# nikolovjovan/exblas

Measured on AMD Instinct MI355X. Metric: ExSUM fp64 Gelem/s at n=2^28 (bit-exact vs CPU superaccumulator/MPFR), higher is better.
Workload: dtype f64; 1 GPU; ExSUM n=2^28 fp64 ill_cond(c=1e+32), fpe=8 early_exit=True, 1xMI355X, inputs resident in HBM, steps rotate over 4 distinct vectors; n_total=268435456, fpe=8, early_exit=True, parallelism=single

## Files before the change

exblas_amd/csrc/blas1.hip:

```cpp
#include "superacc.hip.h"
#include "fpe.hip.h"
#include "exblas_internal.h"
#include <hip/hip_ext.h>

namespace exb {

constexpr int BLOCK = 256;
constexpr int WAVES = BLOCK / 64;
constexpr int U = 4;

template <int N, bool EE, int COPIES, int CNT, int ZM = 0>
__device__ __forceinline__ void fpe_absorb(double (&a)[N > 0 ? N : 1], double (&x)[CNT], int from,
                                           long long *col, unsigned &flags)
{
    LdsSink<COPIES> sink{col, flags};
    fpe_absorb_sink<N, EE, CNT, LdsSink<COPIES>, ZM>(a, x, from, sink);
}

template <int N, int COPIES>
__device__ __forceinline__ void fpe_flush(double (&a)[N > 0 ? N : 1], long long *col, unsigned &flags)
{
    LdsSink<COPIES> sink{col, flags};
    fpe_flush_sink<N>(a, sink);
}

template <int COPIES>
__device__ __forceinline__ void block_epilogue(long long *s_acc, unsigned flags, long long *gacc,
                                               unsigned *gflags, int ngroups)
{
    __shared__ unsigned s_flags;
    if (threadIdx.x == 0) s_flags = 0;
    __syncthreads();
    if (flags) atomicOr(&s_flags, flags);
    long long *g = gacc + (size_t)(blockIdx.x % ngroups) * NL;
    for (int l = threadIdx.x; l < NL; l += BLOCK) {
        long long sum = 0;
#pragma unroll
        for (int w = 0; w < WAVES; ++w)
#pragma unroll
            for (int c = 0; c < COPIES; ++c) sum += s_acc[(w * NL + l) * COPIES + c];
        if (sum != 0) atomicAdd((unsigned long long *)&g[l], (unsigned long long)sum);
    }
    __syncthreads();
    if (threadIdx.x == 0 && s_flags) atomicOr(gflags, s_flags);
}

template <int N, bool EE, int COPIES>
__global__ void __launch_bounds__(BLOCK) k_exsum(const double *__restrict__ a, long long n,
                                                 long long *__restrict__ gacc,
                                                 unsigned *__restrict__ gflags, int ngroups)
{
    __shared__ long long s_acc[WAVES * NL * COPIES];
    auto zero_lds = [&]() {
        for (int i = threadIdx.x; i < WAVES * NL * COPIES; i += BLOCK) s_acc[i] = 0;
        __syncthreads();
    };
    const int wave = threadIdx.x >> 6, lane = threadIdx.x & 63;
    long long *col = s_acc + wave * NL * COPIES + (lane & (COPIES - 1));
    unsigned flags = 0;
    double fpe[N > 0 ? N : 1];
#pragma unroll
    for (int i = 0; i < (N > 0 ? N : 1); ++i) fpe[i] = 0.0;

    const long long head = (((uintptr_t)a & 8u) && n > 0) ? 1 : 0;
    const d2_t *v = (const d2_t *)(a + head);
    const long long nv = (n - head) >> 1;
    constexpr long long TILE = (long long)BLOCK * U;
    const long long ntiles = nv / TILE;
    LdsSink<COPIES> sinkm{col, flags};
    Bypass bypass;

    long long t = blockIdx.x;
    if (t < ntiles) {
        d2_t r0[U], r1[U];
        auto fill = [&](long long tile, d2_t (&r)[U]) {
            const d2_t *p = v + (tile < ntiles ? tile : ntiles - 1) * TILE + threadIdx.x;
#pragma unroll
            for (int u = 0; u < U; ++u) r[u] = ld2(p + u * BLOCK);
        };
        auto absorb = [&](d2_t (&r)[U]) {
            double x[2 * U];
#pragma unroll
            for (int u = 0; u < U; ++u) {
                x[2 * u] = r[u].x;
                x[2 * u + 1] = r[u].y;
            }
            fpe_absorb_adaptive<N, EE, 2 * U, LdsSink<COPIES>>(fpe, x, sinkm, bypass);
        };
        fill(t, r0);
        zero_lds();
        for (;;) {
            fill(t + gridDim.x, r1);
            absorb(r0);
            t += gridDim.x;
            if (t >= ntiles) break;
            fill(t + gridDim.x, r0);
            absorb(r1);
            t += gridDim.x;
            if (t >= ntiles) break;
        }
    } else {
        zero_lds();
    }
    for (long long i = ntiles * TILE + (long long)blockIdx.x * BLOCK + threadIdx.x; i < nv;
         i += (long long)gridDim.x * BLOCK) {
        d2_t r = v[i];
        double x[2] = {r.x, r.y};
        fpe_absorb<N, false, COPIES, 2>(fpe, x, 0, col, flags);
    }
    if (blockIdx.x == 0 && threadIdx.x == 0) {
        if (head) lds_add<COPIES>(col, a[0], flags);
        if ((n - head) & 1) lds_add<COPIES>(col, a[n - 1], flags);
    }
    fpe_flush<N, COPIES>(fpe, col, flags);
    block_epilogue<COPIES>(s_acc, flags, gacc, gflags, ngroups);
}

template <int N, bool EE, int COPIES>
__global__ void __launch_bounds__(BLOCK) k_exsum_strided(const double *__restrict__ a, long long n,
                                                         long long inca, long long *__restrict__ gacc,
                                                         unsigned *__restrict__ gflags, int ngroups)
{
    __shared__ long long s_acc[WAVES * NL * COPIES];
    for (int i = threadIdx.x; i < WAVES * NL * COPIES; i += BLOCK) s_acc[i] = 0;
    __syncthreads();
    const int wave = threadIdx.x >> 6, lane = threadIdx.x & 63;
    long long *col = s_acc + wave * NL * COPIES + (lane & (COPIES - 1));
    unsigned flags = 0;
    double fpe[N > 0 ? N : 1];
#pragma unroll
    for (int i = 0; i < (N > 0 ? N : 1); ++i) fpe[i] = 0.0;
    const long long T = (long long)gridDim.x * BLOCK;
    for (long long i = (long long)blockIdx.x * BLOCK + threadIdx.x; i < n; i += 4 * T) {
        double x[4];
#pragma unroll
        for (int u = 0; u < 4; ++u) x[u] = i + u * T < n ? a[(i + u * T) * inca] : 0.0;
        fpe_absorb<N, false, COPIES, 4>(fpe, x, 0, col, flags);
    }
    fpe_flush<N, COPIES>(fpe, col, flags);
    block_epilogue<COPIES>(s_acc, flags, gacc, gflags, ngroups);
}

template <int N, bool EE, int COPIES, int ZM>
__global__ void __launch_bounds__(BLOCK) k_exdot(const double *__restrict__ a, const double *__restrict__ b,
                                                 long long n, long long *__restrict__ gacc,
                                                 unsigned *__restrict__ gflags, int ngroups)
{
    __shared__ long long s_acc[WAVES * NL * COPIES];
    auto zero_lds = [&]() {
        for (int i = threadIdx.x; i < WAVES * NL * COPIES; i += BLOCK) s_acc[i] = 0;
        __syncthreads();
    };
    const int wave = threadIdx.x >> 6, lane = threadIdx.x & 63;
    long long *col = s_acc + wave * NL * COPIES + (lane & (COPIES - 1));
    unsigned flags = 0;
    LdsSink<COPIES> sink{col, flags};
    long long *const lo_acc = low_acc_of(gflags), *const hi_acc = high_acc_of(gflags);
    double fpe[N > 0 ? N : 1];
#pragma unroll
    for (int i = 0; i < (N > 0 ? N : 1); ++i) fpe[i] = 0.0;

    const d2_t *va = (const d2_t *)a, *vb = (const d2_t *)b;
    const long long nv = n >> 1;
    Bypass bypass;
    constexpr long long TILE = (long long)BLOCK * U;
    const long long ntiles = nv / TILE;
    long long t = blockIdx.x;
    d2_t ra[U], rb[U];
    if (t < ntiles) {
        const long long base = t * TILE + threadIdx.x;
#pragma unroll
        for (int u = 0; u < U; ++u) {
            ra[u] = ld2(va + base + u * BLOCK);
            rb[u] = ld2(vb + base + u * BLOCK);
        }
    }
    zero_lds();
    if (t < ntiles) {
        d2_t rc[U], rd[U];
        auto fill = [&](long long tile, d2_t (&pa)[U], d2_t (&pb)[U]) {
            const long long base = (tile < ntiles ? tile : ntiles - 1) * TILE + threadIdx.x;
#pragma unroll
            for (int u = 0; u < U; ++u) {
                pa[u] = ld2(va + base + u * BLOCK);
                pb[u] = ld2(vb + base + u * BLOCK);
            }
        };
        auto absorb = [&](d2_t (&pa)[U], d2_t (&pb)[U]) {
            double x[2 * U], e[2 * U];
#pragma unroll
            for (int u = 0; u < U; ++u) {
                x[2 * u] = two_prod(pa[u].x, pb[u].x, e[2 * u]);
                x[2 * u + 1] = two_prod(pa[u].y, pb[u].y, e[2 * u + 1]);
            }
            if (!prod_range_divert<2 * U>(fpe[0], x, e, sink, lo_acc, hi_acc, [&](int j) { return j & 1 ? pa[j >> 1].y : pa[j >> 1].x; },
                                              [&](int j) { return j & 1 ? pb[j >> 1].y : pb[j >> 1].x; }))
                fpe_absorb_prod_adaptive<N, EE, 2 * U, LdsSink<COPIES>, ZM, false>(fpe, x, e, sink, bypass);
        };
        for (;;) {
            fill(t + gridDim.x, rc, rd);
            absorb(ra, rb);
            t += gridDim.x;
            if (t >= ntiles) break;
            fill(t + gridDim.x, ra, rb);
            absorb(rc, rd);
            t += gridDim.x;
            if (t >= ntiles) break;
        }
    }
    for (long long i = ntiles * TILE + (long long)blockIdx.x * BLOCK + threadIdx.x; i < nv;
         i += (long long)gridDim.x * BLOCK) {
        d2_t ra = va[i], rb = vb[i];
        double x[2], e[2];
        x[0] = two_prod(ra.x, rb.x, e[0]);
        x[1] = two_prod(ra.y, rb.y, e[1]);
        if (!prod_range_divert<2>(fpe[0], x, e, sink, lo_acc, hi_acc, [&](int j) { return j ? ra.y : ra.x; }, [&](int j) { return j ? rb.y : rb.x; }))
            fpe_absorb_prod<N, false, 2, LdsSink<COPIES>, 0, false>(fpe, x, e, sink);
    }
    if (blockIdx.x == 0 && threadIdx.x == 0 && (n & 1)) {
        double x1[1], e1[1];
        x1[0] = two_prod(a[n - 1], b[n - 1], e1[0]);
        if (!prod_range_divert<1>(fpe[0], x1, e1, sink, lo_acc, hi_acc, [&](int) { return a[n - 1]; }, [&](int) { return b[n - 1]; }))
            sink_product(sink, x1[0], e1[0]);
    }
    fpe_flush<N, COPIES>(fpe, col, flags);
    block_epilogue<COPIES>(s_acc, flags, gacc, gflags, ngroups);
}

template <int N, bool EE, int COPIES>
__global__ void __launch_bounds__(BLOCK) k_exdot_strided(const double *__restrict__ a, long long inca,
                                                         const double *__restrict__ b, long long incb,
                                                         long long n, long long *__restrict__ gacc,
                                                         unsigned *__restrict__ gflags, int ngroups)
{
    __shared__ long long s_acc[WAVES * NL * COPIES];
    for (int i = threadIdx.x; i < WAVES * NL * COPIES; i += BLOCK) s_acc[i] = 0;
    __syncthreads();
    const int wave = threadIdx.x >> 6, lane = threadIdx.x & 63;
    long long *col = s_acc + wave * NL * COPIES + (lane & (COPIES - 1));
    unsigned flags = 0;
    LdsSink<COPIES> sink{col, flags};
    long long *const lo_acc = low_acc_of(gflags), *const hi_acc = high_acc_of(gflags);
    double fpe[N > 0 ? N : 1];
#pragma unroll
    for (int i = 0; i < (N > 0 ? N : 1); ++i) fpe[i] = 0.0;
    const long long T = (long long)gridDim.x * BLOCK;
    for (long long i = (long long)blockIdx.x * BLOCK + threadIdx.x; i < n; i += 4 * T) {
        double va[4], vb[4], x[4], e[4];
#pragma unroll
        for (int u = 0; u < 4; ++u) {
            const bool in = i + u * T < n;
            va[u] = in ? a[(i + u * T) * inca] : 0.0;
            vb[u] = in ? b[(i + u * T) * incb] : 0.0;
        }
#pragma unroll
        for (int u = 0; u < 4; ++u) x[u] = two_prod(va[u], vb[u], e[u]);
        if (!prod_range_divert<4>(fpe[0], x, e, sink, lo_acc, hi_acc, [&](int j) { return va[j]; }, [&](int j) { return vb[j]; }))
            fpe_absorb_prod<N, false, 4, LdsSink<COPIES>, 0, false>(fpe, x, e, sink);
    }
    fpe_flush<N, COPIES>(fpe, col, flags);
    block_epilogue<COPIES>(s_acc, flags, gacc, gflags, ngroups);
}

__global__ void __launch_bounds__(64) k_finalize(long long *sets, int nsets, int set_stride, unsigned *gflags,
                                                 unsigned flags_or, int zero_sets, long long *out,
                                                 const long long *ext_in, long long *ext_out)
{
    const int lane = threadIdx.x;
    unsigned flags = flags_or;
    if (gflags) flags |= *gflags;
    if (set_stride >= SET_WORDS) {
        for (int g = 0; g < nsets; ++g)
        {
            for (int k = 0; k < 3; ++k)
                if (sets[(size_t)g * set_stride + NL + k] != 0) flags |= (1u << k);
            const long long pw = sets[(size_t)g * set_stride + NL + 3];
            if (pw & 0xffff) flags |= FLAG_PUNDER;
            if (pw >> 16) flags |= FLAG_POVER;
        }
    }
    long long lo0 = 0, hi0 = 0, lo1 = 0, hi1 = 0;
    for (int g0 = 0; g0 < nsets; g0 += 16) {
        long long t0[16], t1[16];
#pragma unroll
        for (int k = 0; k < 16; ++k) {
            const bool ok = g0 + k < nsets;
            const long long *p = sets + (size_t)(ok ? g0 + k : 0) * set_stride;
            t0[k] = ok ? __builtin_nontemporal_load(p + lane) : 0;
            t1[k] = (ok && lane < NL - 64) ? __builtin_nontemporal_load(p + 64 + lane) : 0;
        }
#pragma unroll
        for (int k = 0; k < 16; ++k) {
            lo0 += t0[k] & 0xffffffffll;
            hi0 += t0[k] >> 32;
            if (lane == NL - 65) {
                lo1 += t1[k];
            } else {
                lo1 += t1[k] & 0xffffffffll;
                hi1 += t1[k] >> 32;
            }
        }
    }
    long long in0 = __shfl_up(hi0, 1), in1 = __shfl_up(hi1, 1);
    const long long h63 = __shfl(hi0, 63);
    if (lane == 0) { in0 = 0; in1 = h63; }
    long long v0 = lo0 + in0, v1 = (lane < NL - 64) ? lo1 + in1 : 0;
    if (zero_sets) {
        for (int i = lane; i < nsets * set_stride; i += 64) sets[i] = 0;
        if (lane == 0 && gflags) *gflags = 0;
    }
    __shared__ long long s_v[NL], s_lo[NL], s_hi[NL], s_c[NL + EXT_SHIFT_DIGITS];
    __shared__ unsigned long long s_ex;
    __shared__ int s_over;
    bool low_folded = false;
    const bool have_low = (flags & FLAG_PUNDER) && (ext_in || gflags);
    const bool have_high = (flags & FLAG_POVER) && (ext_in || gflags);
    if (ext_out) {
        if (!have_low) {
            ext_out[lane] = 0;
            if (lane < SET_WORDS - 64) ext_out[64 + lane] = 0;
        }
        if (!have_high) {
            ext_out[SET_WORDS + lane] = 0;
            if (lane < SET_WORDS - 64) ext_out[SET_WORDS + 64 + lane] = 0;
        }
    }
    if (have_low || have_high) {
        const long long *lsrc = ext_in ? ext_in : low_acc_of(gflags);
        const long long *hsrc = ext_in ? ext_in + SET_WORDS : high_acc_of(gflags);
        s_lo[lane] = have_low ? lsrc[lane] : 0;
        s_hi[lane] = have_high ? hsrc[lane] : 0;
        s_v[lane] = v0;
        if (lane < NL - 64) {
            s_lo[64 + lane] = have_low ? lsrc[64 + lane] : 0;
            s_hi[64 + lane] = have_high ? hsrc[64 + lane] : 0;
            s_v[64 + lane] = v1;
        }
        if (!ext_in && zero_sets) {
            long long *lo = low_acc_of(gflags), *hi = high_acc_of(gflags);
            if (have_low) {
                lo[lane] = 0;
                if (lane < NL - 64) lo[64 + lane] = 0;
            }
            if (have_high) {
                hi[lane] = 0;
                if (lane < NL - 64) hi[64 + lane] = 0;
            }
        }
        __syncthreads();
        if (lane == 0) {
            s_over = 0;
            if (have_low) normalize_digits(s_lo);
            if (have_high) normalize_digits(s_hi);
            if (!ext_out) {
                if (have_high) s_over = fold_high_digits(s_v, s_hi, s_c);
                if (have_low && !s_over) {
                    for (int j = LOW_SHIFT_DIGITS; j < NL; ++j) s_v[j - LOW_SHIFT_DIGITS] += s_lo[j];
                    normalize_digits(s_v);
                    const bool half = (s_lo[LOW_SHIFT_DIGITS - 1] >> 31) & 1ll;
                    bool sticky = (s_lo[LOW_SHIFT_DIGITS - 1] & 0x7fffffffll) != 0;
                    for (int j = 0; j < LOW_SHIFT_DIGITS - 1; ++j) sticky = sticky || s_lo[j] != 0;
                    s_ex = round_exact_bits_frac(s_v, half, sticky);
                }
            }
        }
        __syncthreads();
        if (ext_out) {
            if (have_low) {
                ext_out[lane] = s_lo[lane];
                if (lane < SET_WORDS - 64) ext_out[64 + lane] = lane < NL - 64 ? s_lo[64 + lane] : 0;
            }
            if (have_high) {
                ext_out[SET_WORDS + lane] = s_hi[lane];
                if (lane < SET_WORDS - 64) ext_out[SET_WORDS + 64 + lane] = lane < NL - 64 ? s_hi[64 + lane] : 0;
            }
        } else {
            const int over = s_over;
            if (over) {
                flags |= over > 0 ? FLAG_PINF : FLAG_NINF;
            } else {
                v0 = s_v[lane];
                v1 = lane < NL - 64 ? s_v[64 + lane] : 0;
                low_folded = have_low;
            }
            if (have_low) flags |= FLAG_PLOW_EXACT;
            if (have_high) flags |= FLAG_PHIGH_EXACT;
        }
    }
    WaveFinish r = finish_wave(v0, v1, flags);
    if (low_folded && !(flags & FLAG_NONFINITE)) r.ex = s_ex;
    write_record_wave(r, flags, out);
}

template <int N, bool EE>
__global__ void __launch_bounds__(BLOCK) k_exsum_segmented(const double *__restrict__ values,
                                                           const long long *__restrict__ offsets, long long nseg,
                                                           int round_mode, double *__restrict__ out)
{
    __shared__ long long acc[WAVES][NL];
    __shared__ unsigned fl[WAVES];
    const int lane = threadIdx.x & 63, w = threadIdx.x >> 6;
    const long long seg = (long long)blockIdx.x * WAVES + w;
    const bool valid = seg < nseg;
    for (int t = lane; t < NL; t += 64) acc[w][t] = 0;
    if (lane == 0) fl[w] = 0;
    __syncthreads();
    if (valid) {
        unsigned flags = 0;
        LdsSink<1> sink{acc[w], flags};
        double fpe[N > 0 ? N : 1];
#pragma unroll
        for (int i = 0; i < (N > 0 ? N : 1); ++i) fpe[i] = 0.0;
        const long long b = offsets[seg], e = offsets[seg + 1];
        for (long long i0 = b; i0 < e; i0 += 64) {
            const long long i = i0 + lane;
            double x[1] = {i < e ? values[i] : 0.0};
            fpe_absorb_sink<N, EE, 1>(fpe, x, 0, sink);
        }
        fpe_flush_sink<N>(fpe, sink);
        if (flags) atomicOr(&fl[w], flags);
    }
    __syncthreads();
    const WaveFinish r = finish_wave(acc[w][lane], lane < NL - 64 ? acc[w][64 + lane] : 0, fl[w]);
    if (valid && lane == 0) out[seg] = round_mode ? r.rf : __longlong_as_double((long long)r.ex);
}

__global__ void __launch_bounds__(BLOCK) k_exsum_segmented_zero(long long nseg, double *__restrict__ out)
{
    for (long long i = (long long)blockIdx.x * BLOCK + threadIdx.x; i < nseg; i += (long long)gridDim.x * BLOCK) out[i] = 0.0;
}


#define EXB_LAUNCH_STREAMING(c, kernel, grid, st, ...)                                                                \
    do {                                                                                                               \
        if ((c).launch_stop_event || (c).launch_start_event) {                                                         \
            hipEvent_t ev0_ = (c).launch_start_event, ev1_ = (c).launch_stop_event;                                    \
            (c).launch_start_event = (c).launch_stop_event = nullptr;                                                  \
            hipExtLaunchKernelGGL(kernel, dim3(grid), dim3(BLOCK), 0, st, ev0_, ev1_, 0, __VA_ARGS__);                 \
        } else {                                                                                                       \
            hipLaunchKernelGGL(kernel, dim3(grid), dim3(BLOCK), 0, st, __VA_ARGS__);                                   \
        }                                                                                                              \
    } while (0)

static inline int grid_for(const Ctx &c, long long work_items, long long per_block, int blocks_per_cu)
{
    long long want = (work_items + per_block - 1) / per_block;
    long long cap = (long long)c.num_cu * blocks_per_cu;
    if (want < 1) want = 1;
    if (want >= cap) return (int)max(1ll, cap + c.grid_adj);
    return (int)want;
}

template <int N, bool EE, int COPIES>
static void run_exsum(Ctx &c, const double *a, long long n, hipStream_t st)
{
    const int bpc = N == 0 ? c.bpc_sa : ((!SKIP_ZERO_LEVELS<EE> && N >= 5) ? c.bpc_heavy : c.bpc_sum);
    int grid = grid_for(c, n, (long long)BLOCK * 2 * U, bpc);
    if (grid == c.num_cu * bpc && grid > 1 && !(grid & 1)) grid -= 1;
    EXB_LAUNCH_STREAMING(c, (k_exsum<N, EE, COPIES>), grid, st, a, n, c.gacc, c.gflags, c.ngroups);
}

#ifndef EXBLAS_SUM_COPIES
#define EXBLAS_SUM_COPIES 8
#endif
#ifndef EXBLAS_DOT_COPIES
#define EXBLAS_DOT_COPIES 8
#endif
template <int N, bool EE>
static hipError_t launch_exsum(Ctx &c, const double *a, long long n, long long inca, hipStream_t st)
{
    constexpr int COPIES = (N == 0) ? 16 : EXBLAS_SUM_COPIES;
    if (inca == 1) {
        run_exsum<N, EE, COPIES>(c, a, n, st);
    } else {
        int grid = grid_for(c, n, BLOCK, c.blocks_per_cu);
        EXB_LAUNCH_STREAMING(c, (k_exsum_strided<N, EE, COPIES>), grid, st, a, n, inca, c.gacc, c.gflags, c.ngroups);
    }
    return hipGetLastError();
}

template <int N, bool EE, int COPIES>
static void run_exdot(Ctx &c, const double *a, const double *b, long long n, hipStream_t st)
{
    const long long tiles = n / ((long long)BLOCK * 2 * U);
    const int bpc = (int)min((long long)c.bpc_dot, max(4ll, tiles / (5ll * c.num_cu)));
    int grid = grid_for(c, n, (long long)BLOCK * 2 * U, bpc);
    if (grid > c.num_cu && !(grid & 1)) grid += 1;
    EXB_LAUNCH_STREAMING(c, (k_exdot<N, EE, COPIES, SKIP_ZERO_LEVELS<EE> ? 1 : 0>), grid, st, a, b, n, c.gacc, c.gflags,
                         c.ngroups);
}

template <int N, bool EE>
static hipError_t launch_exdot(Ctx &c, const double *a, long long inca, const double *b, long long incb,
                               long long n, hipStream_t st)
{
    constexpr int COPIES = (N == 0) ? 16 : EXBLAS_DOT_COPIES;
    const bool vec = inca == 1 && incb == 1 && (((uintptr_t)a | (uintptr_t)b) & 15u) == 0;
    if (vec) {
        run_exdot<N, EE, COPIES>(c, a, b, n, st);
    } else {
        int grid = grid_for(c, n, BLOCK, c.blocks_per_cu);
        EXB_LAUNCH_STREAMING(c, (k_exdot_strided<N, EE, COPIES>), grid, st, a, inca, b, incb, n, c.gacc, c.gflags,
                             c.ngroups);
    }
    return hipGetLastError();
}

hipError_t finalize_groups(Ctx &c, hipStream_t st, long long *d_out, long long *d_ext_out)
{
    hipLaunchKernelGGL(k_finalize, dim3(1), dim3(64), 0, st, c.gacc, c.ngroups, NL, c.gflags, 0u, 1, d_out,
                       (const long long *)nullptr, d_ext_out);
    return hipGetLastError();
}

hipError_t finalize_sets(const long long *d_sets, int nsets, unsigned flags_or, hipStream_t st, long long *d_out,
                         const long long *d_ext_sets)
{
    hipLaunchKernelGGL(k_finalize, dim3(1), dim3(64), 0, st, const_cast<long long *>(d_sets), nsets, SET_WORDS,
                       (unsigned *)nullptr, flags_or, 0, d_out, d_ext_sets, (long long *)nullptr);
    return hipGetLastError();
}

hipError_t exsum_dispatch(Ctx &c, const double *a, long long n, long long inca, int fpe, int early_exit,
                          hipStream_t st)
{
    if (fpe < 2) return launch_exsum<0, false>(c, a, n, inca, st);
    hipError_t e = hipSuccess;
    select_variant<2>(fpe, early_exit, [&](auto N, auto EE) { e = launch_exsum<N(), EE()>(c, a, n, inca, st); });
    return e;
}

hipError_t exsum_segmented_dispatch(const double *values, const long long *offsets, long long nseg, int fpe,
                                    int early_exit, int round_mode, hipStream_t st, double *out)
{
    if (nseg <= 0) return hipSuccess;
    const dim3 grid((unsigned)((nseg + WAVES - 1) / WAVES)), block(BLOCK);
    auto go = [&](auto N, auto EE) {
        hipLaunchKernelGGL((k_exsum_segmented<N(), EE()>), grid, block, 0, st, values, offsets, nseg, round_mode, out);
    };
    if (fpe < 2) go(std::integral_constant<int, 0>(), std::false_type());
    else if (!select_variant<2>(fpe, early_exit, go))
        hipLaunchKernelGGL(k_exsum_segmented_zero, dim3((unsigned)min(4096ll, (nseg + BLOCK - 1) / BLOCK)), block, 0, st, nseg,
                           out);
    return hipGetLastError();
}

hipError_t exdot_dispatch(Ctx &c, const double *a, long long inca, const double *b, long long incb, long long n,
                          int fpe, int early_exit, hipStream_t st)
{
    if (fpe < 3) return launch_exdot<0, false>(c, a, inca, b, incb, n, st);
    hipError_t e = hipSuccess;
    select_variant<3>(fpe, early_exit,
                      [&](auto N, auto EE) { e = launch_exdot<N(), EE()>(c, a, inca, b, incb, n, st); });
    return e;
}

}
```

exblas_amd/csrc/fpe.hip.h:

```cpp
#pragma once
#include "superacc.hip.h"

namespace exb {

typedef double d2_t __attribute__((ext_vector_type(2)));

__device__ __forceinline__ d2_t ld2(const d2_t *p) { return __builtin_nontemporal_load(p); }

__device__ __forceinline__ unsigned expo_field(double x) { return ((unsigned)__double2hiint(x) >> 20) & 0x7ffu; }
constexpr unsigned BIG_EXPO = 1023u + 1000u;
constexpr unsigned LOW_EXPO = 1023u - 968u;

template <int CNT, int ZM = 0>
__device__ __forceinline__ bool any_nonzero(const double (&x)[CNT])
{
    if constexpr (ZM == 0) {
        unsigned bits = 0;
#pragma unroll
        for (int j = 0; j < CNT; ++j)
            bits |= ((unsigned)__double2hiint(x[j]) << 1) | (unsigned)__double2loint(x[j]);
        return bits != 0;
    } else {
        bool nz = false;
#pragma unroll
        for (int j = 0; j < CNT; ++j) nz |= (x[j] != 0.0);
        return nz;
    }
}

template <int COPIES>
struct LdsSink {
    long long *col;
    unsigned &flags;
    __device__ __forceinline__ void add(double x) { lds_add<COPIES>(col, x, flags); }
    __device__ __forceinline__ void note(unsigned bits) { flags |= bits; }
};

struct GlobalSink {
    long long *acc;
    __device__ __forceinline__ void note(unsigned) {}
    __device__ __forceinline__ void add(double x)
    {
        const unsigned long long u = (unsigned long long)__double_as_longlong(x);
        unsigned be = (unsigned)(u >> 52) & 0x7ffu;
        unsigned long long m = u & 0x000fffffffffffffull;
        if (be == 0x7ffu) {
            atomicAdd((unsigned long long *)&acc[NL + (m ? 2 : ((u >> 63) ? 1 : 0))], 1ull);
            return;
        }
        if (be) m |= 0x0010000000000000ull; else be = 1u;
        const unsigned p = be - 1u;
        const unsigned idx = p >> 5, sh = p & 31u;
        const unsigned long long lo = m << sh;
        const unsigned hi = (unsigned)((m >> 32) >> (32u - sh));
        long long c0 = (long long)(lo & 0xffffffffull), c1 = (long long)(lo >> 32), c2 = (long long)hi;
        if (u >> 63) { c0 = -c0; c1 = -c1; c2 = -c2; }
        unsigned long long *q = (unsigned long long *)(acc + idx);
        if (c0) atomicAdd(q, (unsigned long long)c0);
        if (c1) atomicAdd(q + 1, (unsigned long long)c1);
        if (c2) atomicAdd(q + 2, (unsigned long long)c2);
    }
};

template <class Sink>
__device__ __forceinline__ void sink_product(Sink &sink, double p, double e)
{
    sink.add(p);
    if (expo_field(p) != 0x7ffu) {
        if (e != 0.0) sink.add(e);
    } else if (__builtin_isinf(p) && __builtin_isinf(e)) {
        sink.note(FLAG_POVER);
    }
}

template <int CNT, class Sink, class FA, class FB>
__device__ __forceinline__ bool prod_range_divert(double &a0, const double (&p)[CNT], const double (&e)[CNT], Sink &sink,
                                                  long long *lo, long long *hi, FA &&a_of, FB &&b_of)
{
    unsigned mn = 0x7ffu, mx = expo_field(a0);
#pragma unroll
    for (int j = 0; j < CNT; ++j) {
        const unsigned ex = expo_field(p[j]);
        mn = min(mn, ex);
        mx = max(mx, ex);
    }
    if (__builtin_expect(!__any(mn < LOW_EXPO || mx >= BIG_EXPO), 1)) return false;
    bool hz = mx >= BIG_EXPO;
#pragma unroll
    for (int j = 0; j < CNT; ++j) hz |= expo_field(p[j]) < LOW_EXPO && a_of(j) != 0.0 && b_of(j) != 0.0;
    if (!__any(hz)) return false;
    GlobalSink low{lo}, high{hi};
#pragma unroll
    for (int j = 0; j < CNT; ++j) {
        const double a = a_of(j), b = b_of(j);
        const unsigned ex = expo_field(p[j]);
        if (ex < LOW_EXPO && a != 0.0 && b != 0.0) {
            int ea;
            const double a1 = frexp(a, &ea);
            const double b1 = ldexp(b, EXT_SHIFT_BITS + ea);
            const double P = a1 * b1, E = __builtin_fma(a1, b1, -P);
            low.add(P);
            if (E != 0.0) low.add(E);
            sink.note(FLAG_PUNDER);
        } else if (ex == 0x7ffu && expo_field(a) != 0x7ffu && expo_field(b) != 0x7ffu) {
            int ea;
            const double a1 = frexp(a, &ea);
            const double b1 = ldexp(b, ea - EXT_SHIFT_BITS);
            const double P = a1 * b1, E = __builtin_fma(a1, b1, -P);
            high.add(P);
            if (E != 0.0) high.add(E);
            sink.note(FLAG_POVER);
        } else {
            sink_product(sink, p[j], e[j]);
        }
    }
    if (expo_field(a0) >= BIG_EXPO) {
        sink.add(a0);
        a0 = 0.0;
    }
    return true;
}

template <int CNT, class Sink>
__device__ __forceinline__ bool fpe_guard(double &a0, const double (&x)[CNT], const double *e, Sink &sink)
{
    unsigned mx = expo_field(a0);
#pragma unroll
    for (int j = 0; j < CNT; ++j) mx = max(mx, expo_field(x[j]));
    if (__builtin_expect(!__any(mx >= BIG_EXPO), 1)) return false;
#pragma unroll
    for (int j = 0; j < CNT; ++j) {
        if (e) sink_product(sink, x[j], e[j]);
        else sink.add(x[j]);
    }
    if (expo_field(a0) >= BIG_EXPO) {
        sink.add(a0);
        a0 = 0.0;
    }
    return true;
}

#ifndef EXBLAS_FULL_CASCADE
#define EXBLAS_FULL_CASCADE 0
#endif
template <bool EE>
inline constexpr bool SKIP_ZERO_LEVELS = EE || !EXBLAS_FULL_CASCADE;

template <int N, bool EE, int CNT, class Sink, int ZM = 0>
__device__ __forceinline__ bool fpe_cascade(double (&a)[N > 0 ? N : 1], double (&x)[CNT], int from, Sink &sink)
{
    bool live = true;
#pragma unroll
    for (int i = 0; i < N; ++i) {
        if (i >= from && live) {
#pragma unroll
            for (int j = 0; j < CNT; ++j) {
                double s;
                a[i] = two_sum(a[i], x[j], s);
                x[j] = s;
            }
            if (SKIP_ZERO_LEVELS<EE> && i > from) live = __any(any_nonzero<CNT, ZM>(x));
        }
    }
    const bool spill = live && __any(any_nonzero<CNT, ZM>(x));
    if (spill) {
#pragma unroll
        for (int j = 0; j < CNT; ++j)
            if (x[j] != 0.0) sink.add(x[j]);
    }
    return spill;
}

template <int N, bool EE, int CNT, class Sink, int ZM = 0>
__device__ __forceinline__ bool fpe_absorb_sink(double (&a)[N > 0 ? N : 1], double (&x)[CNT], int from, Sink &sink)
{
    if constexpr (N == 0) {
#pragma unroll
        for (int j = 0; j < CNT; ++j) sink.add(x[j]);
        return false;
    } else {
        if (from == 0 && fpe_guard<CNT>(a[0], x, nullptr, sink)) return true;
        return fpe_cascade<N, EE, CNT, Sink, ZM>(a, x, from, sink);
    }
}

#ifndef EXBLAS_BYPASS_MIN
#define EXBLAS_BYPASS_MIN 63
#define EXBLAS_BYPASS_MAX 4095
#endif
constexpr int BYPASS_MIN = EXBLAS_BYPASS_MIN, BYPASS_MAX = EXBLAS_BYPASS_MAX;

struct Bypass {
    int left = 0;
    int span = BYPASS_MIN;
    __device__ __forceinline__ void spilled()
    {
        left = span;
        span = min(2 * span + 1, BYPASS_MAX);
    }
};

template <int N, bool EE, int CNT, class Sink, int ZM = 0>
__device__ __forceinline__ void fpe_absorb_adaptive(double (&a)[N > 0 ? N : 1], double (&x)[CNT], Sink &sink, Bypass &bp)
{
    if constexpr (N == 0) {
        fpe_absorb_sink<N, EE, CNT, Sink, ZM>(a, x, 0, sink);
    } else {
        if (__builtin_expect(bp.left > 0, 0)) {
            --bp.left;
#pragma unroll
            for (int j = 0; j < CNT; ++j) sink.add(x[j]);
        } else if (fpe_absorb_sink<N, EE, CNT, Sink, ZM>(a, x, 0, sink)) {
            bp.spilled();
        } else {
            bp.span = BYPASS_MIN;
        }
    }
}

template <int N, bool EE, int CNT, class Sink, int ZM = 0, bool GUARD = true>
__device__ __forceinline__ bool fpe_absorb_prod(double (&a)[N > 0 ? N : 1], double (&p)[CNT], double (&e)[CNT],
                                                Sink &sink)
{
    if constexpr (N == 0) {
#pragma unroll
        for (int j = 0; j < CNT; ++j) {
            sink_product(sink, p[j], e[j]);
        }
        return false;
    } else {
        constexpr int EFROM = (N >= 3) ? N - 3 : 0;
        if constexpr (GUARD) {
            if (fpe_guard<CNT>(a[0], p, e, sink)) return true;
        }
        const bool s1 = fpe_cascade<N, EE, CNT, Sink, ZM>(a, p, 0, sink);
        const bool s2 = fpe_cascade<N, EE, CNT, Sink, ZM>(a, e, EFROM, sink);
        return s1 || s2;
    }
}

template <int N, bool EE, int CNT, class Sink, int ZM = 0, bool GUARD = true>
__device__ __forceinline__ void fpe_absorb_prod_adaptive(double (&a)[N > 0 ? N : 1], double (&p)[CNT],
                                                         double (&e)[CNT], Sink &sink, Bypass &bp)
{
    if constexpr (N == 0) {
        fpe_absorb_prod<N, EE, CNT>(a, p, e, sink);
    } else {
        if (__builtin_expect(bp.left > 0, 0)) {
            --bp.left;
#pragma unroll
            for (int j = 0; j < CNT; ++j) {
                sink_product(sink, p[j], e[j]);
            }
        } else if (fpe_absorb_prod<N, EE, CNT, Sink, ZM, GUARD>(a, p, e, sink)) {
            bp.spilled();
        } else {
            bp.span = BYPASS_MIN;
        }
    }
}

template <int N, class Sink>
__device__ __forceinline__ void fpe_flush_sink(double (&a)[N > 0 ? N : 1], Sink &sink)
{
    if constexpr (N > 0) {
#pragma unroll
        for (int i = 0; i < N; ++i) {
            if (a[i] != 0.0) sink.add(a[i]);
            a[i] = 0.0;
        }
    }
}

}
```

exblas_amd/csrc/superacc.hip.h:

```cpp
#pragma once
#include <hip/hip_runtime.h>
#include <stdint.h>

namespace exb {

constexpr int NL = 68;
constexpr int CANON = 41;
constexpr int CANON_DIGITS = 52;
constexpr int CANON_FWORDS = 21;

constexpr int OUT_EXACT = 0;
constexpr int OUT_REFMODE = 1;
constexpr int OUT_FLAGS = 2;
constexpr int OUT_CANON = 4;
constexpr int OUT_DIGITS = 48;
constexpr int OUT_FLAGCNT = 116;
constexpr int SET_WORDS = 72;
constexpr int OUT_WORDS = 128;

constexpr unsigned FLAG_PINF = 1u, FLAG_NINF = 2u, FLAG_NAN = 4u;
constexpr unsigned FLAG_PUNDER = 8u, FLAG_POVER = 16u, FLAG_NONFINITE = 7u;
constexpr unsigned FLAG_PLOW_EXACT = 32u, FLAG_PHIGH_EXACT = 64u;
constexpr int EXT_SHIFT_DIGITS = 38, EXT_SHIFT_BITS = 32 * EXT_SHIFT_DIGITS;
constexpr int LOW_SHIFT_DIGITS = EXT_SHIFT_DIGITS, LOW_SHIFT_BITS = EXT_SHIFT_BITS;
constexpr int EXT_WORDS = 2 * SET_WORDS;
constexpr int FLAG_BLOCK_BYTES = 64 + EXT_WORDS * 8;
__device__ __forceinline__ long long *low_acc_of(unsigned *gflags) { return (long long *)((char *)gflags + 64); }
__device__ __forceinline__ long long *high_acc_of(unsigned *gflags) { return low_acc_of(gflags) + SET_WORDS; }

__device__ __forceinline__ double two_sum(double a, double b, double &s)
{
    double r = a + b;
    double z = r - a;
    s = (a - (r - z)) + (b - z);
    return r;
}

__device__ __forceinline__ double two_prod(double a, double b, double &e)
{
    double p = a * b;
    e = __builtin_fma(a, b, -p);
    return p;
}

__device__ __forceinline__ double two_prod_safe(double a, double b, double &e)
{
    double p = a * b;
    double t = __builtin_fma(a, b, -p);
    e = __builtin_isfinite(p) ? t : 0.0;
    return p;
}

template <int COPIES>
__device__ __forceinline__ void lds_add(long long *col, double x, unsigned &flags)
{
    const unsigned long long u = (unsigned long long)__double_as_longlong(x);
    unsigned be = (unsigned)(u >> 52) & 0x7ffu;
    unsigned long long m = u & 0x000fffffffffffffull;
    if (be == 0x7ffu) {
        flags |= m ? FLAG_NAN : ((u >> 63) ? FLAG_NINF : FLAG_PINF);
        return;
    }
    if (be) m |= 0x0010000000000000ull; else be = 1u;
    const unsigned p = be - 1u;
    const unsigned idx = p >> 5, sh = p & 31u;
    const unsigned long long lo = m << sh;
    const unsigned hi = (unsigned)((m >> 32) >> (32u - sh));
    long long c0 = (long long)(lo & 0xffffffffull);
    long long c1 = (long long)(lo >> 32);
    long long c2 = (long long)hi;
    if (u >> 63) { c0 = -c0; c1 = -c1; c2 = -c2; }
    unsigned long long *q = (unsigned long long *)(col + idx * COPIES);
    atomicAdd(q, (unsigned long long)c0);
    atomicAdd(q + COPIES, (unsigned long long)c1);
    atomicAdd(q + 2 * COPIES, (unsigned long long)c2);
}

__device__ inline void normalize_digits(long long *v, int nd = NL)
{
    long long carry = 0;
    for (int i = 0; i < nd - 1; ++i) {
        long long t = v[i] + carry;
        carry = t >> 32;
        v[i] = t & 0xffffffffll;
    }
    v[nd - 1] += carry;
}

__device__ inline int fold_high_digits(long long *v, const long long *h, long long *c)
{
    constexpr int ND = NL + EXT_SHIFT_DIGITS;
    for (int i = 0; i < ND; ++i) c[i] = (i < NL ? v[i] : 0) + (i >= EXT_SHIFT_DIGITS ? h[i - EXT_SHIFT_DIGITS] : 0);
    normalize_digits(c, ND);
    bool zeros = c[ND - 1] == 0, ones = c[ND - 1] == -1;
    for (int i = NL; i < ND - 1; ++i) {
        zeros = zeros && c[i] == 0;
        ones = ones && c[i] == 0xffffffffll;
    }
    if (ones && !((c[NL - 1] >> 31) & 1)) ones = false;
    if (zeros && ((c[NL - 1] >> 31) & 1)) zeros = false;
    if (!zeros && !ones) return c[ND - 1] < 0 ? -1 : 1;
    for (int i = 0; i < NL - 1; ++i) v[i] = c[i];
    v[NL - 1] = zeros ? c[NL - 1] : c[NL - 1] - 0x100000000ll;
    return 0;
}

__device__ inline unsigned long long round_exact_bits(const long long *v)
{
    const bool neg = v[NL - 1] < 0;
    unsigned mag[NL];
    if (!neg) {
        for (int i = 0; i < NL; ++i) mag[i] = (unsigned)v[i];
    } else {
        unsigned long long c = 1;
        for (int i = 0; i < NL; ++i) {
            unsigned long long t = (unsigned long long)(~(unsigned)v[i]) + c;
            mag[i] = (unsigned)t;
            c = t >> 32;
        }
    }
    int t = NL - 1;
    while (t >= 0 && mag[t] == 0) --t;
    const unsigned long long sign = neg ? 0x8000000000000000ull : 0ull;
    if (t < 0) return 0ull;
    const int lz = __builtin_clz(mag[t]);
    const int msb = 32 * t + 31 - lz;
    if (msb <= 52) {
        unsigned long long val = ((unsigned long long)(t >= 1 ? mag[1] : 0u) << 32) | mag[0];
        return sign | val;
    }
    const unsigned d1 = (t >= 1) ? mag[t - 1] : 0u, d2 = (t >= 2) ? mag[t - 2] : 0u;
    unsigned long long w = ((unsigned long long)mag[t] << 32) | d1;
    unsigned rest;
    if (lz) {
        w = (w << lz) | (unsigned long long)(d2 >> (32 - lz));
        rest = d2 << lz;
    } else {
        rest = d2;
    }
    bool sticky = (w & 0x3ffull) != 0 || rest != 0;
    for (int i = t - 3; i >= 0 && !sticky; --i) sticky = mag[i] != 0;
    unsigned long long bits = ((unsigned long long)(msb - 52) << 52) + (w >> 11);
    const bool rnd = (w >> 10) & 1ull;
    if (rnd && (sticky || (bits & 1ull))) bits += 1;
    if ((bits >> 52) >= 0x7ffull) bits = 0x7ff0000000000000ull;
    return sign | bits;
}

__device__ inline unsigned long long round_exact_bits_frac(const long long *v, bool half, bool sticky)
{
    if (!half && !sticky) return round_exact_bits(v);
    const bool neg = v[NL - 1] < 0;
    unsigned mag[NL];
    if (!neg) {
        for (int i = 0; i < NL; ++i) mag[i] = (unsigned)v[i];
    } else {
        for (int i = 0; i < NL; ++i) mag[i] = ~(unsigned)v[i];
        const bool h = half, st = sticky;
        half = !(h && st);
        sticky = !(h && !st);
    }
    const unsigned long long sign = neg ? 0x8000000000000000ull : 0ull;
    int t = NL - 1;
    while (t >= 0 && mag[t] == 0) --t;
    const int lz = t >= 0 ? __builtin_clz(mag[t]) : 0;
    const int msb = t >= 0 ? 32 * t + 31 - lz : -1;
    if (msb <= 52) {
        unsigned long long val = t < 0 ? 0ull : (((unsigned long long)(t >= 1 ? mag[1] : 0u) << 32) | mag[0]);
        if (half && (sticky || (val & 1ull))) val += 1;
        return sign | val;
    }
    const unsigned d1 = (t >= 1) ? mag[t - 1] : 0u, d2 = (t >= 2) ? mag[t - 2] : 0u;
    unsigned long long w = ((unsigned long long)mag[t] << 32) | d1;
    unsigned rest;
    if (lz) {
        w = (w << lz) | (unsigned long long)(d2 >> (32 - lz));
        rest = d2 << lz;
    } else {
        rest = d2;
    }
    bool st2 = true;
    (void)rest;
    unsigned long long bits = ((unsigned long long)(msb - 52) << 52) + (w >> 11);
    const bool rnd = (w >> 10) & 1ull;
    if (rnd && (st2 || (bits & 1ull))) bits += 1;
    if ((bits >> 52) >= 0x7ffull) bits = 0x7ff0000000000000ull;
    return sign | bits;
}

__device__ inline long long digits_field52(const long long *v, int o)
{
    const int q = o >> 5, r = o & 31;
    auto dig = [&](int i) -> unsigned long long {
        if (i < 0) return 0ull;
        if (i >= NL - 1) {
            const long long top = v[NL - 1];
            const int k = i - (NL - 1);
            if (k == 0) return (unsigned long long)(unsigned)top;
            if (k == 1) return (unsigned long long)(unsigned)(top >> 32);
            return (top < 0) ? 0xffffffffull : 0ull;
        }
        return (unsigned long long)(unsigned)v[i];
    };
    const unsigned long long lo = dig(q) | (dig(q + 1) << 32);
    const unsigned long long hi = dig(q + 2) | (dig(q + 3) << 32);
    const unsigned long long win = r ? ((lo >> r) | (hi << (64 - r))) : lo;
    return (long long)(win & ((1ull << CANON_DIGITS) - 1));
}

__device__ inline void digits_to_canon(const long long *v, long long *canon)
{
    for (int j = 0; j < CANON - 1; ++j) canon[j] = digits_field52(v, CANON_DIGITS * j - 18);
    const int o = CANON_DIGITS * (CANON - 1) - 18;
    const int q = o >> 5, r = o & 31;
    auto dig = [&](int i) -> unsigned long long {
        if (i >= NL - 1) {
            const long long top = v[NL - 1];
            const int k = i - (NL - 1);
            if (k == 0) return (unsigned long long)(unsigned)top;
            if (k == 1) return (unsigned long long)(unsigned)(top >> 32);
            return (top < 0) ? 0xffffffffull : 0ull;
        }
        return (unsigned long long)(unsigned)v[i];
    };
    const unsigned long long lo = dig(q) | (dig(q + 1) << 32);
    const unsigned long long hi = dig(q + 2) | (dig(q + 3) << 32);
    canon[CANON - 1] = (long long)(r ? ((lo >> r) | (hi << (64 - r))) : lo);
}

__device__ inline double round_reference(const long long *acc)
{
    const long long mask = (1ll << CANON_DIGITS) - 1;
    const bool negative = acc[CANON - 1] < 0;
    int i;
    for (i = CANON - 1; i >= 0 && acc[i] == 0; --i) { }
    if (negative) {
        for (; i >= 0 && (acc[i] & mask) == mask; --i) { }
    }
    if (i < 0) return 0.0;
    long long hiword = negative ? mask - acc[i] : acc[i];
    double rounded = (double)hiword;
    double hi = ldexp(rounded, (i - CANON_FWORDS) * CANON_DIGITS);
    if (i == 0) return negative ? -hi : hi;
    hiword -= __double2ll_rn(rounded);
    double mid = ldexp((double)hiword, (i - CANON_FWORDS) * CANON_DIGITS);
    long long sticky = 0;
    for (int j = 0; j != i - 1; ++j) sticky |= negative ? (1ll << CANON_DIGITS) - acc[j] : acc[j];
    long long loword = negative ? (1ll << CANON_DIGITS) - acc[i - 1] : acc[i - 1];
    loword |= (sticky != 0);
    double lo = ldexp((double)loword, (i - 1 - CANON_FWORDS) * CANON_DIGITS);
    if (mid != 0) {
        unsigned long long b = (unsigned long long)__double_as_longlong(mid + lo);
        b |= (unsigned long long)(lo != 0.0);
        lo = __longlong_as_double((long long)b);
    }
    hi = hi + lo;
    return negative ? -hi : hi;
}

__device__ inline void finish_record(long long *v, unsigned flags, long long *out)
{
    normalize_digits(v);
    long long canon[CANON];
    digits_to_canon(v, canon);
    unsigned long long ex = round_exact_bits(v);
    double rf = round_reference(canon);
    if (flags & FLAG_NONFINITE) {
        const bool nan = (flags & FLAG_NAN) || ((flags & FLAG_PINF) && (flags & FLAG_NINF));
        ex = nan ? 0x7ff8000000000000ull
                 : ((flags & FLAG_NINF) ? 0xfff0000000000000ull : 0x7ff0000000000000ull);
        rf = __longlong_as_double((long long)ex);
    }
    out[OUT_EXACT] = (long long)ex;
    out[OUT_REFMODE] = __double_as_longlong(rf);
    out[OUT_FLAGS] = (long long)flags;
    out[3] = 0;
    for (int j = 0; j < CANON; ++j) out[OUT_CANON + j] = canon[j];
    for (int j = 0; j < NL; ++j) out[OUT_DIGITS + j] = v[j];
    out[OUT_FLAGCNT + 0] = (flags & FLAG_PINF) ? 1 : 0;
    out[OUT_FLAGCNT + 1] = (flags & FLAG_NINF) ? 1 : 0;
    out[OUT_FLAGCNT + 2] = (flags & FLAG_NAN) ? 1 : 0;
    out[OUT_FLAGCNT + 3] = ((flags & FLAG_PUNDER) ? 1 : 0) + ((flags & FLAG_POVER) ? 65536 : 0);
}

__device__ __forceinline__ long long wave_shr1(long long v)
{
    int lo = (int)v, hi = (int)(v >> 32);
    lo = __builtin_amdgcn_update_dpp(0, lo, 0x138, 0xf, 0xf, true);
    hi = __builtin_amdgcn_update_dpp(0, hi, 0x138, 0xf, 0xf, true);
    return (long long)(((unsigned long long)(unsigned)hi << 32) | (unsigned long long)(unsigned)lo);
}
__device__ __forceinline__ unsigned lane_bcast(unsigned v, int l)
{
    return (unsigned)__builtin_amdgcn_readlane((int)v, l);
}
__device__ __forceinline__ long long lane_bcast(long long v, int l)
{
    const unsigned lo = lane_bcast((unsigned)v, l), hi = lane_bcast((unsigned)(v >> 32), l);
    return (long long)(((unsigned long long)hi << 32) | lo);
}
__device__ __forceinline__ double lane_bcast(double v, int l)
{
    return __longlong_as_double(lane_bcast(__double_as_longlong(v), l));
}

__device__ __forceinline__ void wave_add_double(long long &v0, long long &v1, double x, unsigned &flags)
{
    const int lane = (int)(threadIdx.x & 63u);
    const unsigned long long u = (unsigned long long)__double_as_longlong(x);
    unsigned be = (unsigned)(u >> 52) & 0x7ffu;
    unsigned long long m = u & 0x000fffffffffffffull;
    if (be == 0x7ffu) {
        flags |= m ? FLAG_NAN : ((u >> 63) ? FLAG_NINF : FLAG_PINF);
        return;
    }
    if (be) m |= 0x0010000000000000ull; else be = 1u;
    const unsigned p = be - 1u;
    const int idx = (int)(p >> 5);
    const unsigned sh = p & 31u;
    const unsigned long long lo = m << sh;
    const unsigned hi = (unsigned)((m >> 32) >> (32u - sh));
    long long c0 = (long long)(lo & 0xffffffffull), c1 = (long long)(lo >> 32), c2 = (long long)hi;
    if (u >> 63) { c0 = -c0; c1 = -c1; c2 = -c2; }
    const int k0 = lane - idx;
    const int k1 = lane + 64 - idx;
    v0 += k0 == 0 ? c0 : (k0 == 1 ? c1 : (k0 == 2 ? c2 : 0ll));
    if (lane < NL - 64) v1 += k1 == 0 ? c0 : (k1 == 1 ? c1 : (k1 == 2 ? c2 : 0ll));
}

struct WaveFinish {
    unsigned long long ex;
    double rf;
    long long canon;
    long long d0, d1;
};

template <bool FULL = true>
__device__ inline WaveFinish finish_wave(long long v0, long long v1, const unsigned flags)
{
    const int lane = (int)(threadIdx.x & 63u);
    constexpr int HI = NL - 64;
    if (lane >= HI) v1 = 0;
    const unsigned long long nzA = __ballot(v0 != 0), nzB = __ballot(v1 != 0);
    const int hi = nzB ? 64 + (63 - __builtin_clzll(nzB)) : (nzA ? 63 - __builtin_clzll(nzA) : -1);
    const bool split0 = lane <= hi;
    const bool split1 = (64 + lane <= hi) && (lane < HI - 1);
    for (int pass = 0; pass < 2 * NL && hi >= 0; ++pass) {
        const long long c0 = split0 ? (v0 >> 32) : 0, lo0 = split0 ? (v0 & 0xffffffffll) : v0;
        const long long c1 = split1 ? (v1 >> 32) : 0, lo1 = split1 ? (v1 & 0xffffffffll) : v1;
        long long in0 = wave_shr1(c0), in1 = wave_shr1(c1);
        const long long c63 = lane_bcast(c0, 63);
        if (lane == 0) in1 = c63;
        v0 = lo0 + in0;
        v1 = (lane < HI) ? lo1 + in1 : 0;
        const bool pending = (split0 && (v0 >> 32) != 0) || (split1 && (v1 >> 32) != 0);
        if (!__any(pending)) break;
    }
    if (hi >= 0 && hi + 1 < NL - 1) {
        const int e = hi + 1;
        const long long s0 = lane_bcast(v0, e & 63), s1 = lane_bcast(v1, (e - 64) & 63);
        const long long sv = e < 64 ? s0 : s1;
        const long long fill = sv < 0 ? 0xffffffffll : 0ll;
        if (lane == e) v0 = sv & 0xffffffffll;
        if (lane > e) v0 = fill;
        if (lane < HI) {
            const int i1 = 64 + lane;
            if (i1 == e) v1 = sv & 0xffffffffll;
            if (i1 > e) v1 = (i1 == NL - 1) ? (sv < 0 ? -1ll : 0ll) : fill;
        }
    }
    WaveFinish r;
    r.d0 = v0;
    r.d1 = v1;
    const long long top = lane_bcast(v1, HI - 1);
    const bool neg = top < 0;
    const unsigned d0 = (unsigned)v0, d1 = (unsigned)v1;
    const unsigned long long nz0 = __ballot(d0 != 0), nz1 = __ballot(lane < HI && d1 != 0);
    const int z = nz0 ? __builtin_ctzll(nz0) : (nz1 ? 64 + __builtin_ctzll(nz1) : NL);
// ... 116 lines not shown
```

Before: 860.1 Gelem/s.

## Add branch-free finite LDS sink with wave-level nonfinite check and more copies

Introduces a StreamSink whose spill path decodes each double into three 32-bit digit contributions without branches and adds them to LDS atomically, using 128-bit sign handling. Whole tiles are screened once with a wave-wide any() check for Inf/NaN before taking the fast finite path. Product spills skip the error terms when every lane's errors are zero. LDS accumulator copies are doubled from 8 to 16 to reduce atomic contention, at the cost of more shared memory per block and a longer epilogue reduction.

After: 858.1 Gelem/s. No clear change (-0.2%).

```diff
diff --git a/exblas_amd/csrc/blas1.hip b/exblas_amd/csrc/blas1.hip
--- a/exblas_amd/csrc/blas1.hip
+++ b/exblas_amd/csrc/blas1.hip
@@ -11,17 +11,9 @@
 
 template <int N, bool EE, int COPIES, int CNT, int ZM = 0>
 __device__ __forceinline__ void fpe_absorb(double (&a)[N > 0 ? N : 1], double (&x)[CNT], int from,
-                                           long long *col, unsigned &flags)
-{
-    LdsSink<COPIES> sink{col, flags};
-    fpe_absorb_sink<N, EE, CNT, LdsSink<COPIES>, ZM>(a, x, from, sink);
-}
-
-template <int N, int COPIES>
-__device__ __forceinline__ void fpe_flush(double (&a)[N > 0 ? N : 1], long long *col, unsigned &flags)
-{
-    LdsSink<COPIES> sink{col, flags};
-    fpe_flush_sink<N>(a, sink);
+                                           StreamSink<COPIES> &sink)
+{
+    fpe_absorb_sink<N, EE, CNT, StreamSink<COPIES>, ZM>(a, x, from, sink);
 }
 
 template <int COPIES>
@@ -58,6 +50,7 @@
     const int wave = threadIdx.x >> 6, lane = threadIdx.x & 63;
     long long *col = s_acc + wave * NL * COPIES + (lane & (COPIES - 1));
     unsigned flags = 0;
+    StreamSink<COPIES> sink{col, flags};
     double fpe[N > 0 ? N : 1];
 #pragma unroll
     for (int i = 0; i < (N > 0 ? N : 1); ++i) fpe[i] = 0.0;
@@ -67,7 +60,6 @@
     const long long nv = (n - head) >> 1;
     constexpr long long TILE = (long long)BLOCK * U;
     const long long ntiles = nv / TILE;
-    LdsSink<COPIES> sinkm{col, flags};
     Bypass bypass;
 
     long long t = blockIdx.x;
@@ -85,7 +77,7 @@
                 x[2 * u] = r[u].x;
                 x[2 * u + 1] = r[u].y;
             }
-            fpe_absorb_adaptive<N, EE, 2 * U, LdsSink<COPIES>>(fpe, x, sinkm, bypass);
+            fpe_absorb_adaptive<N, EE, 2 * U>(fpe, x, sink, bypass);
         };
         fill(t, r0);
         zero_lds();
@@ -106,13 +98,13 @@
          i += (long long)gridDim.x * BLOCK) {
         d2_t r = v[i];
         double x[2] = {r.x, r.y};
-        fpe_absorb<N, false, COPIES, 2>(fpe, x, 0, col, flags);
+        fpe_absorb<N, false, COPIES, 2>(fpe, x, 0, sink);
     }
     if (blockIdx.x == 0 && threadIdx.x == 0) {
-        if (head) lds_add<COPIES>(col, a[0], flags);
-        if ((n - head) & 1) lds_add<COPIES>(col, a[n - 1], flags);
-    }
-    fpe_flush<N, COPIES>(fpe, col, flags);
+        if (head) sink.add(a[0]);
+        if ((n - head) & 1) sink.add(a[n - 1]);
+    }
+    fpe_flush_sink<N>(fpe, sink);
     block_epilogue<COPIES>(s_acc, flags, gacc, gflags, ngroups);
 }
 
@@ -127,6 +119,7 @@
     const int wave = threadIdx.x >> 6, lane = threadIdx.x & 63;
     long long *col = s_acc + wave * NL * COPIES + (lane & (COPIES - 1));
     unsigned flags = 0;
+    StreamSink<COPIES> sink{col, flags};
     double fpe[N > 0 ? N : 1];
 #pragma unroll
     for (int i = 0; i < (N > 0 ? N : 1); ++i) fpe[i] = 0.0;
@@ -135,9 +128,9 @@
         double x[4];
 #pragma unroll
         for (int u = 0; u < 4; ++u) x[u] = i + u * T < n ? a[(i + u * T) * inca] : 0.0;
-        fpe_absorb<N, false, COPIES, 4>(fpe, x, 0, col, flags);
-    }
-    fpe_flush<N, COPIES>(fpe, col, flags);
+        fpe_absorb<N, false, COPIES, 4>(fpe, x, 0, sink);
+    }
+    fpe_flush_sink<N>(fpe, sink);
     block_epilogue<COPIES>(s_acc, flags, gacc, gflags, ngroups);
 }
 
@@ -154,7 +147,7 @@
     const int wave = threadIdx.x >> 6, lane = threadIdx.x & 63;
     long long *col = s_acc + wave * NL * COPIES + (lane & (COPIES - 1));
     unsigned flags = 0;
-    LdsSink<COPIES> sink{col, flags};
+    StreamSink<COPIES> sink{col, flags};
     long long *const lo_acc = low_acc_of(gflags), *const hi_acc = high_acc_of(gflags);
     double fpe[N > 0 ? N : 1];
 #pragma unroll
@@ -195,7 +188,7 @@
             }
             if (!prod_range_divert<2 * U>(fpe[0], x, e, sink, lo_acc, hi_acc, [&](int j) { return j & 1 ? pa[j >> 1].y : pa[j >> 1].x; },
                                               [&](int j) { return j & 1 ? pb[j >> 1].y : pb[j >> 1].x; }))
-                fpe_absorb_prod_adaptive<N, EE, 2 * U, LdsSink<COPIES>, ZM, false>(fpe, x, e, sink, bypass);
+                fpe_absorb_prod_adaptive<N, EE, 2 * U, StreamSink<COPIES>, ZM, false>(fpe, x, e, sink, bypass);
         };
         for (;;) {
             fill(t + gridDim.x, rc, rd);
@@ -215,7 +208,7 @@
         x[0] = two_prod(ra.x, rb.x, e[0]);
         x[1] = two_prod(ra.y, rb.y, e[1]);
         if (!prod_range_divert<2>(fpe[0], x, e, sink, lo_acc, hi_acc, [&](int j) { return j ? ra.y : ra.x; }, [&](int j) { return j ? rb.y : rb.x; }))
-            fpe_absorb_prod<N, false, 2, LdsSink<COPIES>, 0, false>(fpe, x, e, sink);
+            fpe_absorb_prod<N, false, 2, StreamSink<COPIES>, 0, false>(fpe, x, e, sink);
     }
     if (blockIdx.x == 0 && threadIdx.x == 0 && (n & 1)) {
         double x1[1], e1[1];
@@ -223,7 +216,7 @@
         if (!prod_range_divert<1>(fpe[0], x1, e1, sink, lo_acc, hi_acc, [&](int) { return a[n - 1]; }, [&](int) { return b[n - 1]; }))
             sink_product(sink, x1[0], e1[0]);
     }
-    fpe_flush<N, COPIES>(fpe, col, flags);
+    fpe_flush_sink<N>(fpe, sink);
     block_epilogue<COPIES>(s_acc, flags, gacc, gflags, ngroups);
 }
 
@@ -239,7 +232,7 @@
     const int wave = threadIdx.x >> 6, lane = threadIdx.x & 63;
     long long *col = s_acc + wave * NL * COPIES + (lane & (COPIES - 1));
     unsigned flags = 0;
-    LdsSink<COPIES> sink{col, flags};
+    StreamSink<COPIES> sink{col, flags};
     long long *const lo_acc = low_acc_of(gflags), *const hi_acc = high_acc_of(gflags);
     double fpe[N > 0 ? N : 1];
 #pragma unroll
@@ -256,9 +249,9 @@
 #pragma unroll
         for (int u = 0; u < 4; ++u) x[u] = two_prod(va[u], vb[u], e[u]);
         if (!prod_range_divert<4>(fpe[0], x, e, sink, lo_acc, hi_acc, [&](int j) { return va[j]; }, [&](int j) { return vb[j]; }))
-            fpe_absorb_prod<N, false, 4, LdsSink<COPIES>, 0, false>(fpe, x, e, sink);
-    }
-    fpe_flush<N, COPIES>(fpe, col, flags);
+            fpe_absorb_prod<N, false, 4, StreamSink<COPIES>, 0, false>(fpe, x, e, sink);
+    }
+    fpe_flush_sink<N>(fpe, sink);
     block_epilogue<COPIES>(s_acc, flags, gacc, gflags, ngroups);
 }
 
@@ -461,10 +454,10 @@
 }
 
 #ifndef EXBLAS_SUM_COPIES
-#define EXBLAS_SUM_COPIES 8
+#define EXBLAS_SUM_COPIES 16
 #endif
 #ifndef EXBLAS_DOT_COPIES
-#define EXBLAS_DOT_COPIES 8
+#define EXBLAS_DOT_COPIES 16
 #endif
 template <int N, bool EE>
 static hipError_t launch_exsum(Ctx &c, const double *a, long long n, long long inca, hipStream_t st)
diff --git a/exblas_amd/csrc/fpe.hip.h b/exblas_amd/csrc/fpe.hip.h
--- a/exblas_amd/csrc/fpe.hip.h
+++ b/exblas_amd/csrc/fpe.hip.h
@@ -33,6 +33,18 @@
     long long *col;
     unsigned &flags;
     __device__ __forceinline__ void add(double x) { lds_add<COPIES>(col, x, flags); }
+    __device__ __forceinline__ void note(unsigned bits) { flags |= bits; }
+};
+
+template <int COPIES>
+struct StreamSink {
+    long long *col;
+    unsigned &flags;
+    __device__ __forceinline__ void add(double x)
+    {
+        if (expo_field(x) == 0x7ffu) flags |= nonfinite_flags(x);
+        else lds_add_finite<COPIES>(col, x);
+    }
     __device__ __forceinline__ void note(unsigned bits) { flags |= bits; }
 };
 
@@ -70,6 +82,57 @@
         if (e != 0.0) sink.add(e);
     } else if (__builtin_isinf(p) && __builtin_isinf(e)) {
         sink.note(FLAG_POVER);
+    }
+}
+
+template <int CNT, class Sink>
+__device__ __forceinline__ void sink_tile(Sink &sink, const double (&x)[CNT])
+{
+#pragma unroll
+    for (int j = 0; j < CNT; ++j) sink.add(x[j]);
+}
+
+template <int CNT, class Sink>
+__device__ __forceinline__ void sink_product_tile(Sink &sink, const double (&p)[CNT], const double (&e)[CNT])
+{
+#pragma unroll
+    for (int j = 0; j < CNT; ++j) sink_product(sink, p[j], e[j]);
+}
+
+template <int CNT>
+__device__ __forceinline__ bool tile_has_nonfinite(const double (&x)[CNT])
+{
+    unsigned mx = 0;
+#pragma unroll
+    for (int j = 0; j < CNT; ++j) mx = max(mx, expo_field(x[j]));
+    return __any(mx == 0x7ffu);
+}
+
+template <int CNT, int COPIES>
+__device__ __forceinline__ void sink_tile(StreamSink<COPIES> &sink, const double (&x)[CNT])
+{
+    if (__builtin_expect(tile_has_nonfinite<CNT>(x), 0)) {
+#pragma unroll
+        for (int j = 0; j < CNT; ++j) sink.add(x[j]);
+    } else {
+#pragma unroll
+        for (int j = 0; j < CNT; ++j) lds_add_finite<COPIES>(sink.col, x[j]);
+    }
+}
+
+template <int CNT, int COPIES>
+__device__ __forceinline__ void sink_product_tile(StreamSink<COPIES> &sink, const double (&p)[CNT], const double (&e)[CNT])
+{
+    if (__builtin_expect(tile_has_nonfinite<CNT>(p), 0)) {
+#pragma unroll
+        for (int j = 0; j < CNT; ++j) sink_product(sink, p[j], e[j]);
+    } else {
+#pragma unroll
+        for (int j = 0; j < CNT; ++j) lds_add_finite<COPIES>(sink.col, p[j]);
+        if (__any(any_nonzero<CNT>(e))) {
+#pragma unroll
+            for (int j = 0; j < CNT; ++j) lds_add_finite<COPIES>(sink.col, e[j]);
+        }
     }
 }
 
@@ -175,8 +238,7 @@
 __device__ __forceinline__ bool fpe_absorb_sink(double (&a)[N > 0 ? N : 1], double (&x)[CNT], int from, Sink &sink)
 {
     if constexpr (N == 0) {
-#pragma unroll
-        for (int j = 0; j < CNT; ++j) sink.add(x[j]);
+        sink_tile<CNT>(sink, x);
         return false;
     } else {
         if (from == 0 && fpe_guard<CNT>(a[0], x, nullptr, sink)) return true;
@@ -208,8 +270,7 @@
     } else {
         if (__builtin_expect(bp.left > 0, 0)) {
             --bp.left;
-#pragma unroll
-            for (int j = 0; j < CNT; ++j) sink.add(x[j]);
+            sink_tile<CNT>(sink, x);
         } else if (fpe_absorb_sink<N, EE, CNT, Sink, ZM>(a, x, 0, sink)) {
             bp.spilled();
         } else {
@@ -223,10 +284,7 @@
                                                 Sink &sink)
 {
     if constexpr (N == 0) {
-#pragma unroll
-        for (int j = 0; j < CNT; ++j) {
-            sink_product(sink, p[j], e[j]);
-        }
+        sink_product_tile<CNT>(sink, p, e);
         return false;
     } else {
         constexpr int EFROM = (N >= 3) ? N - 3 : 0;
@@ -248,10 +306,7 @@
     } else {
         if (__builtin_expect(bp.left > 0, 0)) {
             --bp.left;
-#pragma unroll
-            for (int j = 0; j < CNT; ++j) {
-                sink_product(sink, p[j], e[j]);
-            }
+            sink_product_tile<CNT>(sink, p, e);
         } else if (fpe_absorb_prod<N, EE, CNT, Sink, ZM, GUARD>(a, p, e, sink)) {
             bp.spilled();
         } else {
diff --git a/exblas_amd/csrc/superacc.hip.h b/exblas_amd/csrc/superacc.hip.h
--- a/exblas_amd/csrc/superacc.hip.h
+++ b/exblas_amd/csrc/superacc.hip.h
@@ -74,6 +74,32 @@
     atomicAdd(q, (unsigned long long)c0);
     atomicAdd(q + COPIES, (unsigned long long)c1);
     atomicAdd(q + 2 * COPIES, (unsigned long long)c2);
+}
+
+template <int COPIES>
+__device__ __forceinline__ void lds_add_finite(long long *col, double x)
+{
+    const unsigned h = (unsigned)__double2hiint(x), l = (unsigned)__double2loint(x);
+    const unsigned be = (h >> 20) & 0x7ffu;
+    const unsigned mh = (h & 0x000fffffu) | (((be + 0x7ffu) << 9) & 0x00100000u);
+    const unsigned p = max(be, 1u) - 1u;
+    const unsigned sh = p & 31u;
+    const unsigned long long lo = (((unsigned long long)mh << 32) | l) << sh;
+    const unsigned hi = (mh >> 1) >> (sh ^ 31u);
+    const unsigned long long s = (unsigned long long)(long long)((int)h >> 31);
+    const unsigned __int128 ss = ((unsigned __int128)s << 64) | s;
+    const unsigned __int128 v = ((((unsigned __int128)hi << 64) | lo) ^ ss) - ss;
+    const unsigned long long vl = (unsigned long long)v;
+    unsigned long long *q = (unsigned long long *)((char *)col + (p >> 5) * (COPIES * 8u));
+    atomicAdd(q, vl & 0xffffffffull);
+    atomicAdd(q + COPIES, vl >> 32);
+    atomicAdd(q + 2 * COPIES, (unsigned long long)(long long)(int)(unsigned)(v >> 64));
+}
+
+__device__ __forceinline__ unsigned nonfinite_flags(double x)
+{
+    const unsigned long long u = (unsigned long long)__double_as_longlong(x);
+    return (u & 0x000fffffffffffffull) ? FLAG_NAN : ((u >> 63) ? FLAG_NINF : FLAG_PINF);
 }
 
 __device__ inline void normalize_digits(long long *v, int nd = NL)
```
